# eschnett/RayTraceGR.jl

Measured on AMD Instinct MI355X. Metric: geodesic RK step attempts/s (Tsit5, 6 RHS each), Kerr-Schild screen, whole job, higher is better.
Workload: dtype f64; 1 GPU; example2 scene (Kerr-Schild ks_ref0, 3 objects) 4096x4096 screen, tol=eps^(3/4), lambda in [0,100]; rows dealt cyclic over 1 GPU(s); size=4096, variant=ks_ref0, rhs=closed, entry=device, parallelism=rows/1

## Files before the change

raytracegr.jl_amd/csrc/rtgr_integrate.hpp:

```cpp
#pragma once
#include "rtgr_objects.hpp"
#include "rtgr_tsit5_tables.hpp"

#ifndef RTGR_GHOST_LANES
#define RTGR_GHOST_LANES 1
#endif
#ifndef RTGR_WAVES_PER_SIMD_GENERIC
#define RTGR_WAVES_PER_SIMD_GENERIC 2
#endif
#ifndef RTGR_LDSK_GENERIC
#define RTGR_LDSK_GENERIC 0
#endif
#ifndef RTGR_LDSK_GRID4
#define RTGR_LDSK_GRID4 1
#endif
#ifndef RTGR_LDSK_SPIN_FAR
#define RTGR_LDSK_SPIN_FAR 0
#endif
#ifndef RTGR_WAVES_PER_SIMD_SPIN_FAR
#define RTGR_WAVES_PER_SIMD_SPIN_FAR RTGR_WAVES_PER_SIMD_FAR
#endif
#ifndef RTGR_WAVES_PER_SIMD_GENERIC_F32
#define RTGR_WAVES_PER_SIMD_GENERIC_F32 3
#endif
#ifndef RTGR_WAVES_PER_SIMD_GRID
#define RTGR_WAVES_PER_SIMD_GRID 1
#endif
#ifndef RTGR_WAVES_PER_SIMD_GRID_F32
#define RTGR_WAVES_PER_SIMD_GRID_F32 1
#endif
#ifndef RTGR_WAVES_PER_SIMD_GRID4
#define RTGR_WAVES_PER_SIMD_GRID4 1
#endif
#ifndef RTGR_WAVES_PER_SIMD_GRID4_F32
#define RTGR_WAVES_PER_SIMD_GRID4_F32 1
#endif
#ifndef RTGR_WAVES_PER_SIMD_FAR
#define RTGR_WAVES_PER_SIMD_FAR 3
#endif
#ifndef RTGR_WAVES_PER_SIMD_F32
#define RTGR_WAVES_PER_SIMD_F32 3
#endif
#ifndef RTGR_WAVES_PER_SIMD
#define RTGR_WAVES_PER_SIMD 2
#endif

namespace rtgr {

template <class R, int METRIC, bool SPIN = false> constexpr int waves_per_simd_of(int mode) {
    if (Sampled<R, METRIC>::time_dependent) return sizeof(R) == 8 ? RTGR_WAVES_PER_SIMD_GRID4 : RTGR_WAVES_PER_SIMD_GRID4_F32;
    if (Sampled<R, METRIC>::is) return sizeof(R) == 8 ? RTGR_WAVES_PER_SIMD_GRID : RTGR_WAVES_PER_SIMD_GRID_F32;
    if (METRIC >= RTGR_GENERIC_BASE) return sizeof(R) == 8 ? RTGR_WAVES_PER_SIMD_GENERIC : RTGR_WAVES_PER_SIMD_GENERIC_F32;
    if (mode == MODE_FAR) return sizeof(R) == 8 ? (SPIN ? RTGR_WAVES_PER_SIMD_SPIN_FAR : RTGR_WAVES_PER_SIMD_FAR) : 4;
    return sizeof(R) == 8 ? RTGR_WAVES_PER_SIMD : RTGR_WAVES_PER_SIMD_F32;
}
template <class R, int METRIC, bool SPIN> constexpr bool ldsk_of(int mode) {
    if (Sampled<R, METRIC>::time_dependent) return sizeof(R) == 8 && RTGR_LDSK_GRID4 != 0;
    if (METRIC >= RTGR_GENERIC_BASE) return RTGR_LDSK_GENERIC != 0;
    return SPIN && mode == MODE_FAR && RTGR_LDSK_SPIN_FAR != 0;
}

constexpr uint32_t RTGR_EARLY_BUF = 128;
template <class R>
RTGR_DEV void flush_early(const IntegrateArgs<R>& A, const uint32_t* buf, uint32_t cnt, uint32_t lane) {
    unsigned long long base = 0;
    if (lane == 0) base = atomicAdd(A.ctrl + 6, (unsigned long long)cnt);
    base = uniform64(base);
    for (uint32_t i = lane; i < cnt; i += 64) A.early[base + i] = buf[i];
}

template <class R, int METRIC, bool SPIN, bool NPTS10, int MODE, bool LDSK = false>
RTGR_DEV void integrate_body(const IntegrateArgs<R>& A) {
    using N = Tsit5N<R>;
    const uint32_t lane = threadIdx.x & 63;
    uint64_t n_early = 0;
    if (MODE == MODE_NEAR && A.early) {
        const unsigned long long c = A.ctrl[6];
        n_early = uniform64(c);
    }
    const uint64_t total = A.n + n_early;
    unsigned long long* const queue = (MODE == MODE_NEAR) ? A.ctrl + 1 : A.ctrl;
    const MetricK<R> MK = scene_consts<R, METRIC>(A.sc);
    const R reltol = A.opt.reltol, abstol = A.opt.abstol;
    const R t0 = A.opt.lambda0, t1 = A.opt.lambda1, dtmax = uniform_(A.opt.lambda1 - A.opt.lambda0);
    const float igamma = 1.0f / 0.9f, qmin_inv = 5.0f, qmax_inv = 0.1f;
    const float lq_init = -13.287712379549449f;
    const float beta1 = 0.14f, beta2 = 0.08f;
    const int npts = (int)A.opt.interp_points;
    const R eps = sizeof(R) == 8 ? R(2.220446049250313e-16) : R(1.1920929e-7);
    const R t1_snap = uniform_(t1 - R(16) * eps * rmaxabs<R>(t0, t1));
    const uint32_t mask_shift = A.sc.nobj > 64u ? 32u - (uint32_t)__builtin_clz((A.sc.nobj - 1u) >> 6) : 0u;

    int state = L_FREE;
    bool exhausted = false;
    R x[4], u[4], k0[4];
    R t = t0, dt = R(0), ps = R(0);
    float lq = lq_init;
    uint64_t idx = 0;
    uint32_t nacc = 0, nrej = 0, nacc0 = 0, c_maxnear = 0, safe_streak = 0;
    uint32_t c_rays = 0, c_acc = 0, c_rej = 0, c_ev = 0, c_int = 0, c_nf = 0;
#pragma unroll
    for (int q = 0; q < 4; q++) { x[q] = R(1); u[q] = R(0); k0[q] = R(0); }

    uint64_t q_next = 0, q_end = 0;
    bool first_pop = true;
    bool first_early = true, early_done = false;
    __shared__ uint32_t early_buf[RTGR_EARLY_BUF];
    __shared__ R ldsk_mem[LDSK ? 20 * 64 : 1];
    volatile __attribute__((address_space(3))) R* const ldsk = (__attribute__((address_space(3))) R*)(ldsk_mem + lane);
    uint32_t e_cnt = 0;
#ifdef RTGR_ROOT_STATS
    const unsigned long long dbg_t0 = wall_clock64();
    unsigned long long dbg_iters = 0, dbg_rays = 0;
#endif
    const unsigned long long qchunk = A.queue_chunk;
    const uint32_t n_simd = A.n_simd ? A.n_simd : 1024u;
    const uint32_t n_cls = (gridDim.x + n_simd - 1u) / n_simd;
    const uint32_t my_cls = blockIdx.x / n_simd;
    const bool fair = A.fair_shift != 0u && n_cls > 1u;
    for (;;) {
        if (fair) {
            const uint32_t turn = (my_cls + (uint32_t)(__builtin_readcyclecounter() >> A.fair_shift)) % n_cls;
            switch (turn) {
                case 0: __builtin_amdgcn_s_setprio(3); break;
                case 1: __builtin_amdgcn_s_setprio(2); break;
                case 2: __builtin_amdgcn_s_setprio(1); break;
                default: __builtin_amdgcn_s_setprio(0); break;
            }
        }
        const bool resume = (MODE == MODE_NEAR || A.pick_flag != 0u);
        unsigned long long m_need = __ballot(state == L_FREE);
        while (m_need != 0ull) {
            if (q_next == q_end) {
                if (exhausted) break;
                const unsigned long long first_span = 64ull * gridDim.x;
                if (MODE == MODE_NEAR && !early_done) {
                    const unsigned long long echunk = (n_early * 8ull > A.n) ? qchunk : 64ull;
                    unsigned long long eb = 0;
                    if (first_early) eb = echunk * blockIdx.x;
                    else if (lane == 0) eb = atomicAdd(A.ctrl + 7, echunk) + echunk * gridDim.x;
                    first_early = false;
                    eb = uniform64(eb);
                    if (eb >= n_early) { early_done = true; continue; }
                    q_next = eb;
                    q_end = (eb + echunk) < n_early ? (eb + echunk) : n_early;
                    continue;
                }
                const unsigned long long amount = first_pop ? 64ull : qchunk;
                unsigned long long base = 0;
                if (first_pop) base = 64ull * blockIdx.x;
                else if (lane == 0) base = atomicAdd(queue, amount) + first_span;
                first_pop = false;
                base = uniform64(base);
                base += n_early;
                q_next = base < total ? base : total;
                q_end = (base + amount) < total ? (base + amount) : total;
                if (base + amount >= total) exhausted = true;
                if (q_next == q_end) break;
            }
            const uint64_t avail = q_end - q_next;
            const uint32_t rank = mask_rank(m_need, lane);
            if (state == L_FREE && rank < avail) {
                const uint64_t w = q_next + rank;
                uint64_t id = resume ? w : (A.order ? (uint64_t)A.order[w] : w);
                bool take = true;
                if (resume) {
                    const bool listed = MODE == MODE_NEAR && w < n_early;
                    if (MODE == MODE_NEAR) id = listed ? (uint64_t)A.early[w] : w - n_early;
                    take = A.meta[id * 3 + 2] == (listed ? META_HANDED_EARLY : A.pick_flag);
                }
                if (take) {
                    idx = id;
                    state = L_TAKEN;
                }
            }
            const uint32_t cnt = (uint32_t)__builtin_popcountll(m_need);
            q_next += (cnt < avail) ? cnt : avail;
            m_need = __ballot(state == L_FREE);
        }
#ifdef RTGR_ROOT_STATS
        dbg_iters++;
        dbg_rays += __builtin_popcountll(__ballot(state == L_TAKEN));
#endif
        if (state == L_TAKEN) {
            const R* hd = A.hand + idx * HAND_W;
#pragma unroll
            for (int q = 0; q < 4; q++) { x[q] = hd[q]; u[q] = hd[4 + q]; k0[q] = hd[8 + q]; }
            t = hd[12]; dt = hd[13]; ps = hd[14]; lq = (float)hd[15];
            nacc = resume ? A.meta[idx * 3] : 0u;
            nrej = resume ? A.meta[idx * 3 + 1] : 0u;
            nacc0 = nacc;
            safe_streak = 0;
            state = L_RUN;
        }
        if (exhausted && q_next == q_end && state == L_FREE) state = L_EXIT;
        if (__ballot(state == L_RUN) == 0ull) break;

        const bool run = (state == L_RUN);
        bool commit = false;
        bool list_it = false;
        R xn[4], un[4], k[7][4];
#define KL(l, q) ((LDSK && (l) >= 1 && (l) <= 5) ? (R)ldsk[(((l) - 1) * 4 + (q)) * 64] : k[l][q])
#define KSTORE(l)                                                                   \
        if constexpr (LDSK) {                                                       \
            _Pragma("unroll") for (int q_ = 0; q_ < 4; q_++) ldsk[(((l) - 1) * 4 + q_) * 64] = k[l][q_]; \
        }
#pragma unroll
        for (int q = 0; q < 4; q++) k[0][q] = k0[q];
        {
            if (run) dt = rmin(dt, t1 - t);
            const R h = run ? dt : R(0);
            const R h2 = h * h;
            R X[3], U[4];
            constexpr bool TDEP = needs_stage_time<METRIC>();
            R Xt = R(0);
            {
                const R ha = h * N::a[1][0], hc = h * N::c[1];
#pragma unroll
                for (int q = 0; q < 4; q++) U[q] = rfma(ha, k[0][q], u[q]);
#pragma unroll
                for (int q = 0; q < 3; q++) X[q] = rfma(hc, u[1 + q], x[1 + q]);
                if constexpr (TDEP) Xt = rfma(hc, u[0], x[0]);
            }
            accel<R, METRIC, SPIN, true>(X, U, MK, k[1], Xt);
            KSTORE(1);
            {
                const R w1 = h * N::a[2][1], w0 = h * N::a[2][0], hc = h * N::c[2], h2a = h2 * N::A2[2][0];
#pragma unroll
                for (int q = 0; q < 4; q++) U[q] = rfma(w1, KL(1, q), rfma(w0, k[0][q], u[q]));
#pragma unroll
                for (int q = 0; q < 3; q++) X[q] = rfma(h2a, k[0][1 + q], rfma(hc, u[1 + q], x[1 + q]));
                if constexpr (TDEP) Xt = rfma(h2a, k[0][0], rfma(hc, u[0], x[0]));
            }
            accel<R, METRIC, SPIN, true>(X, U, MK, k[2], Xt);
            KSTORE(2);
#pragma unroll
            for (int q = 0; q < 4; q++)
                U[q] = rfma(h, rfma(N::a[3][2], KL(2, q), rfma(N::a[3][1], KL(1, q), N::a[3][0] * k[0][q])), u[q]);
#pragma unroll
            for (int q = 0; q < 3; q++)
                X[q] = rfma(h2, rfma(N::A2[3][1], KL(1, 1 + q), N::A2[3][0] * k[0][1 + q]),
                            rfma(h * N::c[3], u[1 + q], x[1 + q]));
            if constexpr (TDEP) Xt = rfma(h2, rfma(N::A2[3][1], KL(1, 0), N::A2[3][0] * k[0][0]), rfma(h * N::c[3], u[0], x[0]));
            accel<R, METRIC, SPIN, true>(X, U, MK, k[3], Xt);
            KSTORE(3);
#pragma unroll
            for (int q = 0; q < 4; q++)
                U[q] = rfma(h, rfma(N::a[4][3], KL(3, q), rfma(N::a[4][2], KL(2, q), rfma(N::a[4][1], KL(1, q),
                            N::a[4][0] * k[0][q]))), u[q]);
#pragma unroll
            for (int q = 0; q < 3; q++)
                X[q] = rfma(h2, rfma(N::A2[4][2], KL(2, 1 + q), rfma(N::A2[4][1], KL(1, 1 + q), N::A2[4][0] * k[0][1 + q])),
                            rfma(h * N::c[4], u[1 + q], x[1 + q]));
            if constexpr (TDEP) Xt = rfma(h2, rfma(N::A2[4][2], KL(2, 0), rfma(N::A2[4][1], KL(1, 0), N::A2[4][0] * k[0][0])),
                                          rfma(h * N::c[4], u[0], x[0]));
            accel<R, METRIC, SPIN, true>(X, U, MK, k[4], Xt);
            KSTORE(4);
#pragma unroll
            for (int q = 0; q < 4; q++)
                U[q] = rfma(h, rfma(N::a[5][4], KL(4, q), rfma(N::a[5][3], KL(3, q), rfma(N::a[5][2], KL(2, q),
                            rfma(N::a[5][1], KL(1, q), N::a[5][0] * k[0][q])))), u[q]);
#pragma unroll
            for (int q = 0; q < 3; q++)
                X[q] = rfma(h2, rfma(N::A2[5][3], KL(3, 1 + q), rfma(N::A2[5][2], KL(2, 1 + q), rfma(N::A2[5][1], KL(1, 1 + q),
                            N::A2[5][0] * k[0][1 + q]))), rfma(h * N::c[5], u[1 + q], x[1 + q]));
            if constexpr (TDEP) Xt = rfma(h2, rfma(N::A2[5][3], KL(3, 0), rfma(N::A2[5][2], KL(2, 0), rfma(N::A2[5][1], KL(1, 0),
                                          N::A2[5][0] * k[0][0]))), rfma(h * N::c[5], u[0], x[0]));
            accel<R, METRIC, SPIN, true>(X, U, MK, k[5], Xt);
            KSTORE(5);
#pragma unroll
            for (int q = 0; q < 4; q++) {
                un[q] = rfma(h, rfma(N::a[6][5], KL(5, q), rfma(N::a[6][4], KL(4, q), rfma(N::a[6][3], KL(3, q),
                             rfma(N::a[6][2], KL(2, q), rfma(N::a[6][1], KL(1, q), N::a[6][0] * k[0][q]))))), u[q]);
                xn[q] = rfma(h2, rfma(N::A2[6][4], KL(4, q), rfma(N::A2[6][3], KL(3, q), rfma(N::A2[6][2], KL(2, q),
                             rfma(N::A2[6][1], KL(1, q), N::A2[6][0] * k[0][q])))), rfma(h * N::c[6], u[q], x[q]));
            }
            accel<R, METRIC, SPIN, true>(xn + 1, un, MK, k[6], xn[0]);

            if (RTGR_GHOST_LANES ? true : run) {
                float2_t acc2 = {0.0f, 0.0f};
#pragma unroll
                for (int q = 0; q < 4; q++) {
                    const R eu = rfma(N::bt[6], k[6][q], rfma(N::bt[5], KL(5, q), rfma(N::bt[4], KL(4, q),
                                     rfma(N::bt[3], KL(3, q), rfma(N::bt[2], KL(2, q), rfma(N::bt[1], KL(1, q), N::bt[0] * k[0][q]))))));
                    const R ex = rfma(h, rfma(N::BT2[5], KL(5, q), rfma(N::BT2[4], KL(4, q), rfma(N::BT2[3], KL(3, q),
                                     rfma(N::BT2[2], KL(2, q), rfma(N::BT2[1], KL(1, q), N::BT2[0] * k[0][q]))))), N::sbt * u[q]);
                    const float2_t isk = {__builtin_amdgcn_rcpf((float)rfma(rmaxabs<R>(u[q], un[q]), reltol, abstol)),
                                          __builtin_amdgcn_rcpf((float)rfma(rmaxabs<R>(x[q], xn[q]), reltol, abstol))};
                    const float2_t e = {(float)eu, (float)ex};
                    const float2_t r2 = e * isk;
                    acc2 = __builtin_elementwise_fma(r2, r2, acc2);
                }
                const float hf32 = (float)h;
                const float EEst2 = ((acc2.x + acc2.y) * hf32) * (0.125f * hf32);
                uint32_t done = 0xffu;
                bool is_event = false, is_interior = false, handed = false, hand_back = false;
                R top = R(0);
                R cc[4][4];
                bool start_outside = false;
                if constexpr (Sampled<R, METRIC>::is) start_outside = !Sampled<R, METRIC>::inside(MK, x);
                if (start_outside) {
                    done = RTGR_RAY_OUTSIDE;
                } else if (EEst2 != EEst2) {
                    done = RTGR_RAY_NAN;
                } else {
                    const float le = 0.5f * flog2(fmax1(EEst2, 1e-37f));
                    float qf = fexp2(__builtin_fmaf(beta1, le, -beta2 * lq)) * igamma;
                    qf = (EEst2 == 0.0f) ? qmax_inv : fclamp1(qf, qmax_inv, qmin_inv);
                    bool hand_over = false;
                    bool need_scan = true;
                    unsigned long long scan_mask = ~0ull;
                    uint32_t ncand = RTGR_EARLY_BUF + 1u;
                    if constexpr (MODE == MODE_FAR || MODE == MODE_NEAR) {
                        if (EEst2 <= 1.0f) {
                            R dl[4];
#pragma unroll
                            for (int q = 0; q < 4; q++) {
                                R acc2 = N::beta[0] * rabs(k[0][q]);
#pragma unroll
                                for (int l = 1; l < 6; l++) acc2 = rfma(N::beta[l], rabs(KL(l, q)), acc2);
                                dl[q] = h * rfma(h, acc2, rabs(u[q]));
                            }
                            bool safe = true;
                            const R guard = R(1) + R(1e-6);
                            if constexpr (MODE == MODE_NEAR) {
                                scan_mask = __ballot(run && !(ps > R(0))) != 0ull ? ~0ull : 0ull;
                                ncand = scan_mask != 0ull ? RTGR_EARLY_BUF + 1u : 0u;
                            }
                            auto note = [&](bool safe_o, uint32_t o) {
                                safe = safe && safe_o;
                                if constexpr (MODE == MODE_NEAR) {
                                    if (__ballot(run && !safe_o) != 0ull) {
                                        scan_mask |= 1ull << (o >> mask_shift);
                                        if (__builtin_expect(mask_shift != 0u, 0)) {
                                            if (ncand < RTGR_EARLY_BUF) early_buf[ncand] = o;
                                            ncand++;
                                        }
                                    }
                                }
                            };
                            bool group_out = false, run_out = false;
                            for_each_within_reach<R>(A.sc,
                              [&](const DevObject<R>& G, int level) -> bool {
                                R D0, B, mag;
                                sphere_reach<R>(G, x, dl, D0, B, mag);
                                const bool out = D0 > rfma(guard, B, R(256) * eps * mag);
                                if (level != 0) { run_out = out; group_out = out; }
                                else group_out = run_out || out;
                                return __ballot(run && !group_out) != 0ull;
                              },
                              [&](const DevObject<R>& ob, uint32_t o) {
                                R D0, B, mag;
                                sphere_reach<R>(ob, x, dl, D0, B, mag);
                                note(group_out || rabs(D0) > rfma(guard, B, R(256) * eps * mag), o);
                              },
                              [&](const DevObject<R>& ob, uint32_t o) {
                                bool safe_o;
                                if (ob.kind == RTGR_PLANE) {
                                    safe_o = (rabs(x[0] - ob.p[0]) > rfma(guard, dl[0], R(256) * eps * (rabs(x[0]) + rabs(ob.p[0]))));
#ifdef RTGR_USER_OBJECTS
                                } else if (ob.kind == RTGR_USER_OBJECT) {
#ifdef RTGR_USER_REACH
                                    const R gd[4] = {guard * dl[0], guard * dl[1], guard * dl[2], guard * dl[3]};
                                    const R du = rtgr_user_distance<R>(ob.type, x, ob.p);
                                    const R bu = rtgr_user_reach<R>(ob.type, x, ob.p, gd);
                                    safe_o = (rabs(du) > bu + R(256) * eps * (R(1) + rabs(du)));
#else
                                    safe_o = false;
#endif
#endif
                                } else {
                                    R px = x[1], py = x[2];
                                    asm volatile("" : "+v"(px), "+v"(py));
                                    safe_o = (rabs(disk_distance_fast<R>(ob, px, py, x[3])) > guard * rmax(dl[3], dl[1] + dl[2]));
                                }
                                note(safe_o, o);
                              });
                            if constexpr (MODE == MODE_FAR) hand_over = run && (!safe || (ps == R(0)));
                            else {
                                need_scan = !safe || (ps == R(0));
                                safe_streak = need_scan ? 0u : safe_streak + 1u;
                            }
                        }
                        if constexpr (MODE == MODE_NEAR) {
                            need_scan = __ballot(run && (EEst2 <= 1.0f) && need_scan) != 0ull;
                            const unsigned long long m_acc = __ballot(EEst2 <= 1.0f);
                            scan_mask = uniform64(__shfl(scan_mask, m_acc != 0ull ? (int)__builtin_ctzll(m_acc) : 0, 64));
                            ncand = (uint32_t)__builtin_amdgcn_readfirstlane((int)__shfl((int)ncand, m_acc != 0ull ? (int)__builtin_ctzll(m_acc) : 0, 64));
                        }
                    }
                    if (hand_over) {
                        hand_store<R>(A.hand + idx * HAND_W, x, u, k[0], t, dt, ps, lq);
                        const bool early_ray = MODE == MODE_FAR && A.early && nacc < A.near_early;
                        A.meta[idx * 3] = nacc; A.meta[idx * 3 + 1] = nrej;
                        A.meta[idx * 3 + 2] = early_ray ? META_HANDED_EARLY : META_HANDED;
                        if (early_ray) list_it = true;
                        handed = true;
                    } else if (EEst2 <= 1.0f) {
                        nacc++;
                        lq = fmax1(le, lq_init);
                        const R dtnew = dt * (R)__builtin_amdgcn_rcpf(qf);
                        R tnew = t + dt;
                        if (tnew > t1_snap) {
                            if (rabs(tnew - t1) < R(10) * eps * rmaxabs<R>(tnew, t1)) tnew = t1;
                        }
                        if (MODE != MODE_FAR && need_scan) {
#pragma unroll
                        for (int q = 0; q < 4; q++) {
                            cc[0][q] = h * u[q];
#pragma unroll
                            for (int m = 1; m < 4; m++)
                                cc[m][q] = h2 * rfma(N::R2[5][m], KL(5, q), rfma(N::R2[4][m], KL(4, q), rfma(N::R2[3][m], KL(3, q),
                                                rfma(N::R2[2][m], KL(2, q), rfma(N::R2[1][m], KL(1, q), N::R2[0][m] * k[0][q])))));
                        }
                        bool found = false;
                        R nextc;
                        auto scan_objects = [&](auto&& fs, auto&& fo) {
                            if constexpr (MODE == MODE_NEAR) {
                                if (__builtin_expect(mask_shift != 0u && ncand <= RTGR_EARLY_BUF, 0)) {
                                    typedef const DevObject<R> __attribute__((address_space(4))) * ConstTable;
                                    const ConstTable table = (ConstTable)(unsigned long long)(A.sc.more - (uint32_t)RTGR_MAX_OBJECTS);
                                    for (uint32_t c_ = 0; c_ < ncand; c_++) {
                                        const uint32_t o = (uint32_t)__builtin_amdgcn_readfirstlane((int)early_buf[c_]);
                                        if (o < A.sc.nsph) fs(*(const DevObject<R>*)(table + o), o);
                                        else fo(*(const DevObject<R>*)(table + o), o);
                                    }
                                    return;
                                }
                            }
                            for_each_masked_by_kind<R>(A.sc, scan_mask, mask_shift, fs, fo);
                        };
                        if constexpr (NPTS10) {
                            {
                                R pos[5][4], dmin[5];
#pragma unroll
                                for (int j = 0; j < 5; j++) {
                                    const R th = R(j + 1) / R(9);
                                    dmin[j] = R(__builtin_huge_val());
#pragma unroll
                                    for (int q = 0; q < 4; q++)
                                        pos[j][q] = rfma(th, rfma(th, rfma(th, rfma(th, cc[3][q], cc[2][q]), cc[1][q]), cc[0][q]), x[q]);
                                }
                                scan_objects(
                                    [&](const DevObject<R>& ob, uint32_t) { fold_sphere<R, 5>(ob, pos, dmin); },
                                    [&](const DevObject<R>& ob, uint32_t) { fold_distances<R, 5>(ob, pos, dmin); });
#pragma unroll
                                for (int j = 0; j < 5; j++) {
                                    const bool hit = (ps * dmin[j] < R(0)) && !found;
                                    top = hit ? R(j + 1) / R(9) : top;
                                    found = found || hit;
                                }
                            }
                            {
                                R pos[4][4], dmin[4];
#pragma unroll
                                for (int j = 0; j < 3; j++) {
                                    const R th = R(j + 6) / R(9);
                                    dmin[j] = R(__builtin_huge_val());
#pragma unroll
                                    for (int q = 0; q < 4; q++)
                                        pos[j][q] = rfma(th, rfma(th, rfma(th, rfma(th, cc[3][q], cc[2][q]), cc[1][q]), cc[0][q]), x[q]);
                                }
                                dmin[3] = R(__builtin_huge_val());
#pragma unroll
                                for (int q = 0; q < 4; q++) pos[3][q] = xn[q];
                                scan_objects(
                                    [&](const DevObject<R>& ob, uint32_t) { fold_sphere<R, 4>(ob, pos, dmin); },
                                    [&](const DevObject<R>& ob, uint32_t) { fold_distances<R, 4>(ob, pos, dmin); });
                                nextc = dmin[3];
#pragma unroll
                                for (int j = 0; j < 3; j++) {
                                    const bool hit = (ps * dmin[j] < R(0)) && !found;
                                    top = hit ? R(j + 6) / R(9) : top;
                                    found = found || hit;
                                }
                            }
                        } else {
                            nextc = min_distance<R>(A.sc, xn);
                            const R dth = npts > 1 ? R(1) / R(npts - 1) : R(1);
                            for (int j = 1; j + 1 < npts; j++) {
                                const R th = R(j) * dth;
                                R xi[4];
#pragma unroll
                                for (int q = 0; q < 4; q++)
                                    xi[q] = rfma(th, rfma(th, rfma(th, rfma(th, cc[3][q], cc[2][q]), cc[1][q]), cc[0][q]), x[q]);
                                const bool hit = (ps * min_distance<R>(A.sc, xi) < R(0)) && !found;
                                top = hit ? th : top;
                                found = found || hit;
                            }
                        }
                        const bool endpoint = (ps != R(0)) && (ps * nextc <= R(0));
                        found = found && (ps != R(0)) && !endpoint;
                        if (endpoint || found) {
                            top = endpoint ? R(1) : top;
                            is_event = true;
                            is_interior = found;
                            done = RTGR_RAY_EVENT;
                        }
                        if (!is_event) ps = rsign(nextc);
                        }
                        if (!is_event) {
                            commit = true;
                            t = tnew;
                            dt = rmin(dtmax, dtnew);
                            bool outside = false;
                            if constexpr (Sampled<R, METRIC>::is) outside = !Sampled<R, METRIC>::inside(MK, xn);
                            if (outside) done = RTGR_RAY_OUTSIDE;
                            else if (!(t < t1)) done = RTGR_RAY_LAMBDA1;
                            else if (nacc + nrej >= A.opt.max_steps) done = RTGR_RAY_MAXSTEPS;
                            else if (!(t + dt > t)) done = RTGR_RAY_DTMIN;
                            else if (MODE == MODE_NEAR && A.allow_handback && safe_streak >= 2u && (nacc - nacc0) >= A.handback_after) hand_back = true;
                        }
                    } else {
                        nrej++;
                        dt = dt * (R)__builtin_amdgcn_rcpf(fmin1(qmin_inv, fexp2(beta1 * le) * igamma));
                        if (nacc + nrej >= A.opt.max_steps) done = RTGR_RAY_MAXSTEPS;
                        else if (!(t + dt > t)) done = RTGR_RAY_DTMIN;
                    }
                }
                if (!run) {
                    done = 0xffu; is_event = false; is_interior = false; handed = false; hand_back = false; commit = false;
                    list_it = false;
                }
                const bool want_state = (A.recw == REC_TAIL_STATE);
                if (is_event) {
                    const RecRef<R> rec{A.hand + idx * HAND_W, A.rec + idx * (uint64_t)A.recw};
#pragma unroll
                    for (int q = 0; q < 4; q++) rec[REC_X + q] = x[q];
#pragma unroll
                    for (int m = 0; m < 4; m++)
#pragma unroll
                        for (int q = 0; q < 4; q++) rec[REC_C + 4 * m + q] = cc[m][q];
                    rec[REC_PS] = ps;
                    rec[REC_TOP] = top;
                    rec[REC_T] = t;
                    rec[REC_H] = h;
                    if (want_state) {
#pragma unroll
                        for (int q = 0; q < 4; q++) {
                            rec[REC_U + q] = u[q];
#pragma unroll
                            for (int m = 0; m < 4; m++)
                                rec[REC_CU + 4 * m + q] = h * rfma(N::r[6][m], k[6][q], rfma(N::r[5][m], KL(5, q),
                                    rfma(N::r[4][m], KL(4, q), rfma(N::r[3][m], KL(3, q), rfma(N::r[2][m], KL(2, q),
                                    rfma(N::r[1][m], KL(1, q), N::r[0][m] * k[0][q]))))));
                        }
                    }
                }
                if (handed) state = L_FREE;
                if (hand_back) {
                    hand_store<R>(A.hand + idx * HAND_W, xn, un, k[6], t, dt, ps, lq);
                    A.meta[idx * 3] = nacc; A.meta[idx * 3 + 1] = nrej; A.meta[idx * 3 + 2] = META_HANDBACK;
                    if (MODE == MODE_NEAR) c_maxnear = c_maxnear > (nacc - nacc0) ? c_maxnear : (nacc - nacc0);
                    state = L_FREE;
                }
                if (done != 0xffu) {
                    if (!is_event) {
                        const RecRef<R> rec{A.hand + idx * HAND_W, A.rec + idx * (uint64_t)A.recw};
#pragma unroll
                        for (int q = 0; q < 4; q++) rec[REC_X + q] = commit ? xn[q] : x[q];
                        rec[REC_PS] = R(0);
                        rec[REC_TOP] = R(0);
                        rec[REC_T] = t;
                        rec[REC_H] = R(0);
                        if (want_state) {
#pragma unroll
                            for (int q = 0; q < 4; q++) rec[REC_U + q] = commit ? un[q] : u[q];
                        }
                    }
                    uint32_t* mt = A.meta + idx * 3;
                    mt[0] = nacc;
                    mt[1] = nrej;
                    mt[2] = done | (is_interior ? 0x100u : 0u);
                    if (MODE == MODE_NEAR) c_maxnear = c_maxnear > (nacc - nacc0) ? c_maxnear : (nacc - nacc0);
#ifdef RTGR_ROOT_STATS
                    if (MODE == MODE_NEAR && A.dbg) {
                        uint32_t* pr = (uint32_t*)(A.dbg + 4ull * 8192) + 2 * idx;
                        pr[0] = nacc0; pr[1] = nacc - nacc0;
                    }
#endif
                    if constexpr (MODE == MODE_FAR) {
                        if (A.counters) {
                            atomicAdd(&A.counters[0], 1ull);
                            atomicAdd(&A.counters[1], (unsigned long long)nacc);
                            atomicAdd(&A.counters[2], (unsigned long long)nrej);
                            atomicAdd(&A.counters[3], 6ull * (nacc + nrej) + 2ull);
                            if (done >= RTGR_RAY_MAXSTEPS) atomicAdd(&A.counters[6], 1ull);
                        }
                    } else {
                        c_rays += 1; c_acc += nacc; c_rej += nrej;
                        c_ev += is_event; c_int += is_interior; c_nf += (done >= RTGR_RAY_MAXSTEPS);
                    }
                    state = L_FREE;
                }
            }
        }
        if (commit) {
#pragma unroll
            for (int q = 0; q < 4; q++) { x[q] = xn[q]; u[q] = un[q]; k0[q] = k[6][q]; }
        }
        if constexpr (MODE == MODE_FAR) {
            const unsigned long long m_list = __ballot(list_it);
            if (m_list != 0ull) {
                if (list_it) early_buf[e_cnt + mask_rank(m_list, lane)] = (uint32_t)idx;
                e_cnt += (uint32_t)__builtin_popcountll(m_list);
                if (e_cnt > RTGR_EARLY_BUF / 2) { flush_early(A, early_buf, e_cnt, lane); e_cnt = 0; }
            }
        }
    }
    if constexpr (MODE == MODE_FAR) {
        if (e_cnt != 0u) flush_early(A, early_buf, e_cnt, lane);
    }
#ifdef RTGR_ROOT_STATS
    if (A.dbg && lane == 0) {
        unsigned long long* d = A.dbg + 4ull * blockIdx.x;
        d[0] = dbg_t0; d[1] = wall_clock64(); d[2] = dbg_iters; d[3] = dbg_rays;
    }
#endif
    if (MODE != MODE_FAR && A.counters) {
        const unsigned long long s0 = wave_sum(c_rays), s1 = wave_sum(c_acc), s2 = wave_sum(c_rej),
                                 s4 = wave_sum(c_ev), s5 = wave_sum(c_int), s6 = wave_sum(c_nf);
        if (lane == 0) {
            atomicAdd(&A.counters[0], s0);
            atomicAdd(&A.counters[1], s1);
            atomicAdd(&A.counters[2], s2);
            atomicAdd(&A.counters[3], 6ull * (s1 + s2) + 2ull * s0);
            atomicAdd(&A.counters[4], s4);
            atomicAdd(&A.counters[5], s5);
            atomicAdd(&A.counters[6], s6);
        }
        if (MODE == MODE_NEAR) {
            unsigned long long mx = c_maxnear;
#pragma unroll
            for (int off = 32; off > 0; off >>= 1) { const unsigned long long o = __shfl_down(mx, off, 64); mx = mx > o ? mx : o; }
            if (lane == 0) atomicMax(&A.counters[7], mx);
        }
    }
}

#undef KL
#undef KSTORE
template <class R, int METRIC, bool SPIN, bool NPTS10, int MODE>
__global__ __launch_bounds__(64, (waves_per_simd_of<R, METRIC, SPIN>(MODE)))
void integrate_kernel(const IntegrateArgs<R> A) {
    integrate_body<R, METRIC, SPIN, NPTS10, MODE, ldsk_of<R, METRIC, SPIN>(MODE)>(A);
}

template <class R, int METRIC>
__global__ __launch_bounds__(64, 4) void integrate_far4_kernel(const IntegrateArgs<R> A) {
    integrate_body<R, METRIC, false, true, MODE_FAR>(A);
}

}
```

Baseline: 41.18 billion RK step attempts/s.

## Skip per-step queue service and bookkeeping with a single wave-uniform fast-path test

```diff
diff --git a/raytracegr.jl_amd/csrc/rtgr_integrate.hpp b/raytracegr.jl_amd/csrc/rtgr_integrate.hpp
--- a/raytracegr.jl_amd/csrc/rtgr_integrate.hpp
+++ b/raytracegr.jl_amd/csrc/rtgr_integrate.hpp
@@ -43,6 +43,10 @@
 #endif
 #ifndef RTGR_WAVES_PER_SIMD
 #define RTGR_WAVES_PER_SIMD 2
+#endif
+
+#ifndef RTGR_SVC_FAIR
+#define RTGR_SVC_FAIR 0
 #endif
 
 namespace rtgr {
@@ -97,7 +101,7 @@
     R t = t0, dt = R(0), ps = R(0);
     float lq = lq_init;
     uint64_t idx = 0;
-    uint32_t nacc = 0, nrej = 0, nacc0 = 0, c_maxnear = 0, safe_streak = 0;
+    uint32_t nacc = 0, nrej = 0, nacc0 = 0, c_maxnear = 0, safe_streak = 0, ps_zero = 0;
     uint32_t c_rays = 0, c_acc = 0, c_rej = 0, c_ev = 0, c_int = 0, c_nf = 0;
 #pragma unroll
     for (int q = 0; q < 4; q++) { x[q] = R(1); u[q] = R(0); k0[q] = R(0); }
@@ -114,6 +118,8 @@
     unsigned long long dbg_iters = 0, dbg_rays = 0;
 #endif
     const unsigned long long qchunk = A.queue_chunk;
+    bool service = true;
+    constexpr bool ONE_TEST = METRIC < RTGR_GENERIC_BASE;
     const uint32_t n_simd = A.n_simd ? A.n_simd : 1024u;
     const uint32_t n_cls = (gridDim.x + n_simd - 1u) / n_simd;
     const uint32_t my_cls = blockIdx.x / n_simd;
@@ -129,6 +135,7 @@
             }
         }
         const bool resume = (MODE == MODE_NEAR || A.pick_flag != 0u);
+        if (service) {
         unsigned long long m_need = __ballot(state == L_FREE);
         while (m_need != 0ull) {
             if (q_next == q_end) {
@@ -179,7 +186,6 @@
             m_need = __ballot(state == L_FREE);
         }
 #ifdef RTGR_ROOT_STATS
-        dbg_iters++;
         dbg_rays += __builtin_popcountll(__ballot(state == L_TAKEN));
 #endif
         if (state == L_TAKEN) {
@@ -187,6 +193,7 @@
 #pragma unroll
             for (int q = 0; q < 4; q++) { x[q] = hd[q]; u[q] = hd[4 + q]; k0[q] = hd[8 + q]; }
             t = hd[12]; dt = hd[13]; ps = hd[14]; lq = (float)hd[15];
+            if constexpr (MODE == MODE_FAR) ps_zero = (ps == R(0)) ? 1u : 0u;
             nacc = resume ? A.meta[idx * 3] : 0u;
             nrej = resume ? A.meta[idx * 3 + 1] : 0u;
             nacc0 = nacc;
@@ -195,10 +202,17 @@
         }
         if (exhausted && q_next == q_end && state == L_FREE) state = L_EXIT;
         if (__ballot(state == L_RUN) == 0ull) break;
+        }
+#ifdef RTGR_ROOT_STATS
+        dbg_iters++;
+#endif
 
         const bool run = (state == L_RUN);
         bool commit = false;
         bool list_it = false;
+        R t_n = t, dt_n = dt;
+        float lq_n = lq;
+        const uint32_t nacc_n = nacc + 1u;
         R xn[4], un[4], k[7][4];
 #define KL(l, q) ((LDSK && (l) >= 1 && (l) <= 5) ? (R)ldsk[(((l) - 1) * 4 + (q)) * 64] : k[l][q])
 #define KSTORE(l)                                                                   \
@@ -277,6 +291,14 @@
             }
             accel<R, METRIC, SPIN, true>(xn + 1, un, MK, k[6], xn[0]);
 
+            uint32_t done = 0xffu;
+            bool is_event = false, is_interior = false, handed = false, hand_back = false;
+            bool start_outside = false, hand_over = false;
+            bool acc = false;
+            bool leaves = false;
+            float EEst2 = 0.0f, le = 0.0f;
+            R top = R(0);
+            R cc[4][4];
             if (RTGR_GHOST_LANES ? true : run) {
                 float2_t acc2 = {0.0f, 0.0f};
 #pragma unroll
@@ -292,27 +314,18 @@
                     acc2 = __builtin_elementwise_fma(r2, r2, acc2);
                 }
                 const float hf32 = (float)h;
-                const float EEst2 = ((acc2.x + acc2.y) * hf32) * (0.125f * hf32);
-                uint32_t done = 0xffu;
-                bool is_event = false, is_interior = false, handed = false, hand_back = false;
-                R top = R(0);
-                R cc[4][4];
-                bool start_outside = false;
+                EEst2 = ((acc2.x + acc2.y) * hf32) * (0.125f * hf32);
                 if constexpr (Sampled<R, METRIC>::is) start_outside = !Sampled<R, METRIC>::inside(MK, x);
-                if (start_outside) {
-                    done = RTGR_RAY_OUTSIDE;
-                } else if (EEst2 != EEst2) {
-                    done = RTGR_RAY_NAN;
-                } else {
-                    const float le = 0.5f * flog2(fmax1(EEst2, 1e-37f));
+                {
+                    le = 0.5f * flog2(fmax1(EEst2, 1e-37f));
                     float qf = fexp2(__builtin_fmaf(beta1, le, -beta2 * lq)) * igamma;
                     qf = (EEst2 == 0.0f) ? qmax_inv : fclamp1(qf, qmax_inv, qmin_inv);
-                    bool hand_over = false;
+                    const bool acc0 = !start_outside && EEst2 <= 1.0f;
                     bool need_scan = true;
                     unsigned long long scan_mask = ~0ull;
                     uint32_t ncand = RTGR_EARLY_BUF + 1u;
                     if constexpr (MODE == MODE_FAR || MODE == MODE_NEAR) {
-                        if (EEst2 <= 1.0f) {
+                        if (acc0) {
                             R dl[4];
 #pragma unroll
                             for (int q = 0; q < 4; q++) {
@@ -376,34 +389,25 @@
                                 }
                                 note(safe_o, o);
                               });
-                            if constexpr (MODE == MODE_FAR) hand_over = run && (!safe || (ps == R(0)));
+                            if constexpr (MODE == MODE_FAR) hand_over = run && (!safe || ps_zero != 0u);
                             else {
                                 need_scan = !safe || (ps == R(0));
                                 safe_streak = need_scan ? 0u : safe_streak + 1u;
                             }
                         }
                         if constexpr (MODE == MODE_NEAR) {
-                            need_scan = __ballot(run && (EEst2 <= 1.0f) && need_scan) != 0ull;
-                            const unsigned long long m_acc = __ballot(EEst2 <= 1.0f);
+                            need_scan = __ballot(run && acc0 && need_scan) != 0ull;
+                            const unsigned long long m_acc = __ballot(acc0);
                             scan_mask = uniform64(__shfl(scan_mask, m_acc != 0ull ? (int)__builtin_ctzll(m_acc) : 0, 64));
                             ncand = (uint32_t)__builtin_amdgcn_readfirstlane((int)__shfl((int)ncand, m_acc != 0ull ? (int)__builtin_ctzll(m_acc) : 0, 64));
                         }
                     }
-                    if (hand_over) {
-                        hand_store<R>(A.hand + idx * HAND_W, x, u, k[0], t, dt, ps, lq);
-                        const bool early_ray = MODE == MODE_FAR && A.early && nacc < A.near_early;
-                        A.meta[idx * 3] = nacc; A.meta[idx * 3 + 1] = nrej;
-                        A.meta[idx * 3 + 2] = early_ray ? META_HANDED_EARLY : META_HANDED;
-                        if (early_ray) list_it = true;
-                        handed = true;
-                    } else if (EEst2 <= 1.0f) {
-                        nacc++;
-                        lq = fmax1(le, lq_init);
-                        const R dtnew = dt * (R)__builtin_amdgcn_rcpf(qf);
-                        R tnew = t + dt;
-                        if (tnew > t1_snap) {
-                            if (rabs(tnew - t1) < R(10) * eps * rmaxabs<R>(tnew, t1)) tnew = t1;
-                        }
+                    acc = acc0 && !hand_over;
+                    const R dtnew = dt * (R)__builtin_amdgcn_rcpf(qf);
+                    t_n = t + dt;
+                    dt_n = rmin(dtmax, dtnew);
+                    lq_n = fmax1(le, lq_init);
+                    if (acc) {
                         if (MODE != MODE_FAR && need_scan) {
 #pragma unroll
                         for (int q = 0; q < 4; q++) {
@@ -495,28 +499,63 @@
                             top = endpoint ? R(1) : top;
                             is_event = true;
                             is_interior = found;
-                            done = RTGR_RAY_EVENT;
                         }
                         if (!is_event) ps = rsign(nextc);
                         }
-                        if (!is_event) {
-                            commit = true;
-                            t = tnew;
-                            dt = rmin(dtmax, dtnew);
-                            bool outside = false;
-                            if constexpr (Sampled<R, METRIC>::is) outside = !Sampled<R, METRIC>::inside(MK, xn);
-                            if (outside) done = RTGR_RAY_OUTSIDE;
-                            else if (!(t < t1)) done = RTGR_RAY_LAMBDA1;
-                            else if (nacc + nrej >= A.opt.max_steps) done = RTGR_RAY_MAXSTEPS;
-                            else if (!(t + dt > t)) done = RTGR_RAY_DTMIN;
-                            else if (MODE == MODE_NEAR && A.allow_handback && safe_streak >= 2u && (nacc - nacc0) >= A.handback_after) hand_back = true;
-                        }
+                    }
+                    if constexpr (Sampled<R, METRIC>::is) leaves = !Sampled<R, METRIC>::inside(MK, xn);
+                }
+            }
+            unsigned long long m_svc = __ballot(!run || !acc || is_event || leaves) | __ballot(!(t_n < t1_snap)) |
+                                       __ballot(nacc_n + nrej >= A.opt.max_steps) | __ballot(!(t_n + dt_n > t_n));
+            if constexpr (MODE == MODE_NEAR) {
+                if (A.allow_handback) m_svc |= __ballot(safe_streak >= 2u && (nacc_n - nacc0) >= A.handback_after);
+            }
+            service = !ONE_TEST || (RTGR_SVC_FAIR && fair) || uniform64(m_svc) != 0ull;
+            uint32_t nacc_r = nacc;
+            R t_r = t;
+            if (!service) {
+                commit = true;
+            } else {
+                if (start_outside) {
+                    done = RTGR_RAY_OUTSIDE;
+                } else if (EEst2 != EEst2) {
+                    done = RTGR_RAY_NAN;
+                } else if (hand_over) {
+                    if constexpr (MODE == MODE_FAR) {
+                        R* hd = A.hand + idx * HAND_W;
+#pragma unroll
+                        for (int q = 0; q < 4; q++) { hd[q] = x[q]; hd[4 + q] = u[q]; hd[8 + q] = k[0][q]; }
+                        hd[12] = t; hd[13] = dt; hd[15] = (R)lq;
                     } else {
-                        nrej++;
-                        dt = dt * (R)__builtin_amdgcn_rcpf(fmin1(qmin_inv, fexp2(beta1 * le) * igamma));
-                        if (nacc + nrej >= A.opt.max_steps) done = RTGR_RAY_MAXSTEPS;
-                        else if (!(t + dt > t)) done = RTGR_RAY_DTMIN;
-                    }
+                        hand_store<R>(A.hand + idx * HAND_W, x, u, k[0], t, dt, ps, lq);
+                    }
+                    const bool early_ray = MODE == MODE_FAR && A.early && nacc < A.near_early;
+                    A.meta[idx * 3] = nacc; A.meta[idx * 3 + 1] = nrej;
+                    A.meta[idx * 3 + 2] = early_ray ? META_HANDED_EARLY : META_HANDED;
+                    if (early_ray) list_it = true;
+                    handed = true;
+                } else if (EEst2 <= 1.0f) {
+                    nacc_r = nacc_n;
+                    if (t_n > t1_snap) {
+                        if (rabs(t_n - t1) < R(10) * eps * rmaxabs<R>(t_n, t1)) t_n = t1;
+                    }
+                    if (is_event) {
+                        done = RTGR_RAY_EVENT;
+                    } else {
+                        commit = true;
+                        t_r = t_n;
+                        if (leaves) done = RTGR_RAY_OUTSIDE;
+                        else if (!(t_n < t1)) done = RTGR_RAY_LAMBDA1;
+                        else if (nacc_n + nrej >= A.opt.max_steps) done = RTGR_RAY_MAXSTEPS;
+                        else if (!(t_n + dt_n > t_n)) done = RTGR_RAY_DTMIN;
+                        else if (MODE == MODE_NEAR && A.allow_handback && safe_streak >= 2u && (nacc_n - nacc0) >= A.handback_after) hand_back = true;
+                    }
+                } else {
+                    nrej++;
+                    dt = dt * (R)__builtin_amdgcn_rcpf(fmin1(qmin_inv, fexp2(beta1 * le) * igamma));
+                    if (nacc + nrej >= A.opt.max_steps) done = RTGR_RAY_MAXSTEPS;
+                    else if (!(t + dt > t)) done = RTGR_RAY_DTMIN;
                 }
                 if (!run) {
                     done = 0xffu; is_event = false; is_interior = false; handed = false; hand_back = false; commit = false;
@@ -549,9 +588,9 @@
                 }
                 if (handed) state = L_FREE;
                 if (hand_back) {
-                    hand_store<R>(A.hand + idx * HAND_W, xn, un, k[6], t, dt, ps, lq);
-                    A.meta[idx * 3] = nacc; A.meta[idx * 3 + 1] = nrej; A.meta[idx * 3 + 2] = META_HANDBACK;
-                    if (MODE == MODE_NEAR) c_maxnear = c_maxnear > (nacc - nacc0) ? c_maxnear : (nacc - nacc0);
+                    hand_store<R>(A.hand + idx * HAND_W, xn, un, k[6], t_n, dt_n, ps, lq_n);
+                    A.meta[idx * 3] = nacc_n; A.meta[idx * 3 + 1] = nrej; A.meta[idx * 3 + 2] = META_HANDBACK;
+                    if (MODE == MODE_NEAR) c_maxnear = c_maxnear > (nacc_n - nacc0) ? c_maxnear : (nacc_n - nacc0);
                     state = L_FREE;
                 }
                 if (done != 0xffu) {
@@ -561,7 +600,7 @@
                         for (int q = 0; q < 4; q++) rec[REC_X + q] = commit ? xn[q] : x[q];
                         rec[REC_PS] = R(0);
                         rec[REC_TOP] = R(0);
-                        rec[REC_T] = t;
+                        rec[REC_T] = t_r;
                         rec[REC_H] = R(0);
                         if (want_state) {
 #pragma unroll
@@ -569,43 +608,44 @@
                         }
                     }
                     uint32_t* mt = A.meta + idx * 3;
-                    mt[0] = nacc;
+                    mt[0] = nacc_r;
                     mt[1] = nrej;
                     mt[2] = done | (is_interior ? 0x100u : 0u);
-                    if (MODE == MODE_NEAR) c_maxnear = c_maxnear > (nacc - nacc0) ? c_maxnear : (nacc - nacc0);
+                    if (MODE == MODE_NEAR) c_maxnear = c_maxnear > (nacc_r - nacc0) ? c_maxnear : (nacc_r - nacc0);
 #ifdef RTGR_ROOT_STATS
                     if (MODE == MODE_NEAR && A.dbg) {
                         uint32_t* pr = (uint32_t*)(A.dbg + 4ull * 8192) + 2 * idx;
-                        pr[0] = nacc0; pr[1] = nacc - nacc0;
+                        pr[0] = nacc0; pr[1] = nacc_r - nacc0;
                     }
 #endif
                     if constexpr (MODE == MODE_FAR) {
                         if (A.counters) {
                             atomicAdd(&A.counters[0], 1ull);
-                            atomicAdd(&A.counters[1], (unsigned long long)nacc);
+                            atomicAdd(&A.counters[1], (unsigned long long)nacc_r);
                             atomicAdd(&A.counters[2], (unsigned long long)nrej);
-                            atomicAdd(&A.counters[3], 6ull * (nacc + nrej) + 2ull);
+                            atomicAdd(&A.counters[3], 6ull * (nacc_r + nrej) + 2ull);
                             if (done >= RTGR_RAY_MAXSTEPS) atomicAdd(&A.counters[6], 1ull);
                         }
                     } else {
-                        c_rays += 1; c_acc += nacc; c_rej += nrej;
+                        c_rays += 1; c_acc += nacc_r; c_rej += nrej;
                         c_ev += is_event; c_int += is_interior; c_nf += (done >= RTGR_RAY_MAXSTEPS);
                     }
                     state = L_FREE;
                 }
-            }
-        }
-        if (commit) {
+                if constexpr (MODE == MODE_FAR) {
+                    const unsigned long long m_list = __ballot(list_it);
+                    if (m_list != 0ull) {
+                        if (list_it) early_buf[e_cnt + mask_rank(m_list, lane)] = (uint32_t)idx;
+                        e_cnt += (uint32_t)__builtin_popcountll(m_list);
+                        if (e_cnt > RTGR_EARLY_BUF / 2) { flush_early(A, early_buf, e_cnt, lane); e_cnt = 0; }
+                    }
+                }
+            }
+        }
+        if (commit || (RTGR_GHOST_LANES && !run)) {
 #pragma unroll
             for (int q = 0; q < 4; q++) { x[q] = xn[q]; u[q] = un[q]; k0[q] = k[6][q]; }
-        }
-        if constexpr (MODE == MODE_FAR) {
-            const unsigned long long m_list = __ballot(list_it);
-            if (m_list != 0ull) {
-                if (list_it) early_buf[e_cnt + mask_rank(m_list, lane)] = (uint32_t)idx;
-                e_cnt += (uint32_t)__builtin_popcountll(m_list);
-                if (e_cnt > RTGR_EARLY_BUF / 2) { flush_early(A, early_buf, e_cnt, lane); e_cnt = 0; }
-            }
+            t = t_n; dt = dt_n; lq = lq_n; nacc = nacc_n;
         }
     }
     if constexpr (MODE == MODE_FAR) {
```

Result: no change. 41.56 billion RK step attempts/s (median of 6 runs) (+0.9%).
